# BaptisteHudyma/RGB-D-SLAM

Measured on AMD Instinct MI355X. Metric: depth frames/s primitive extraction (640x480), higher is better.
Workload: dtype f64; 1 GPU; 640x480 synthetic planar-room depth stream, plane extraction only (BASELINE.json configs[1]); stream_frames=4096, unique_frames_per_gpu=4096, scene=room, sub_batches=0, frames_rendered_on=device (torch)

## Files before the change

profiles/a1_inventory.py:

```python
#!/usr/bin/env python3
import argparse
import os
import re
import subprocess
import sys

sys.path.insert(0, os.path.dirname(os.path.abspath(__file__)))
from valu_issue import CSRC, RATE_NS, classify

SYMBOLS = (("f32", "_ZN4cape24cape_cell_moments_kernelILb0EEEvNS_12StageAParamsE"),
           ("u16", "_ZN4cape24cape_cell_moments_kernelILb1EEEvNS_12StageAParamsE"))
ORDER = ("prologue", "first trips", "loop trip", "last trips", "partial store", "reduce wave", "scan waves", "scan f64 redo", "aux store")
WEIGHT = {"prologue": 1, "first trips": 1, "loop trip": 3, "last trips": 1, "partial store": 1, "reduce wave": 0.2, "scan waves": 0.8,
          "scan f64 redo": 0.0, "aux store": 0.8}


def find(body, lo, pred):
    return next(i for i in range(lo, len(body)) if pred(body[i]))


def regions(asm, symbol):
    start = next(i for i, ln in enumerate(asm) if ln.startswith(symbol + ":"))
    end = find(asm, start, lambda ln: "s_endpgm" in ln)
    body = asm[start + 1:end + 1]
    is_depth_load = lambda ln: re.search(r"global_load_dwordx[24] .* nt$", ln.rstrip()) is not None
    first_load = find(body, 0, is_depth_load)
    head = find(body, 0, lambda ln: "Loop Header" in ln)
    label = body[head].split(":")[0]
    loop_end = find(body, head, lambda ln: re.search(r"s_c?branch\w*\s+" + re.escape(label) + r"\b", ln) is not None)
    skip = re.search(r"s_cbranch_execz\s+(\S+)", body[find(body, 0, lambda ln: "s_cbranch_execz" in ln)]).group(1)
    join = find(body, loop_end, lambda ln: ln.startswith(skip + ":"))
    barrier = find(body, join, lambda ln: "s_barrier" in ln)
    out = {"prologue": body[:first_load], "first trips": body[first_load:head], "loop trip": body[head:loop_end + 1],
           "last trips": body[loop_end + 1:join], "partial store": body[join:barrier + 1]}
    br = find(body, barrier, lambda ln: re.search(r"s_cbranch_\w+\s+\.LBB", ln) is not None)
    target = re.search(r"(\.LBB\w+)", body[br]).group(1)
    split = find(body, br, lambda ln: ln.startswith(target + ":"))
    arms = [body[barrier + 1:split], body[split:]]
    reduce_arm = next(a for a in arms if any("global_store_dwordx2" in ln for ln in a))
    scan_arm = next(a for a in arms if a is not reduce_arm)
    out["reduce wave"] = reduce_arm
    last_perm = max(i for i, ln in enumerate(scan_arm) if "ds_bpermute_b32" in ln)
    scan, redo = scan_arm[:last_perm + 1], []
    for i, ln in enumerate(scan):
        m = re.search(r"s_cbranch_vccz\s+(\.LBB\w+)", ln)
        if m:
            j = find(scan, i, lambda x: x.startswith(m.group(1) + ":"))
            if any(re.search(r"v_cmp_\w+_f64", x) for x in scan[i:j]):
                scan, redo = scan[:i + 1] + scan[j:], scan[i + 1:j]
                break
    out["scan waves"], out["scan f64 redo"], out["aux store"] = scan, redo, scan_arm[last_perm + 1:]
    return out


def count(lines):
    c = {"f64": 0, "double_rate": 0, "other": 0}
    for ln in lines:
        m = re.match(r"\s+(v_\w+)", ln)
        if m:
            c[classify(m.group(1))] += 1
    return c


def inventory(asm):
    res = {}
    for variant, symbol in SYMBOLS:
        res[variant] = {name: count(lines) for name, lines in regions(asm, symbol).items()}
    return res


def priced(c):
    return sum(c[k] * RATE_NS[k] for k in RATE_NS)


def main():
    ap = argparse.ArgumentParser()
    ap.add_argument("--asm", default="")
    args = ap.parse_args()
    path = args.asm
    if not path:
        path = "/tmp/cape_cell_moments.inventory.s"
        flags = "-O3 -std=c++17 -fPIC --offload-arch=gfx950 -ffp-contract=off -fno-fast-math -fno-slp-vectorize".split()
        subprocess.check_call(["/opt/rocm/bin/hipcc"] + flags + ["-S", "--cuda-device-only", "-o", path, os.path.join(CSRC, "cape_cell_moments.hip")],
                              stderr=subprocess.DEVNULL)
    inv = inventory(open(path).read().splitlines())
    for variant, regs in inv.items():
        print(f"{variant}   VALU instructions as listed                      f64-rate  double-rate  other   total   runs/wave   issue ns/wave")
        tot_n = tot_ns = 0.0
        for name in ORDER:
            c = regs[name]
            n = c["f64"] + c["double_rate"] + c["other"]
            ns = priced(c) * WEIGHT[name]
            tot_n += n * WEIGHT[name]
            tot_ns += ns
            print(f"  {name:<48} {c['f64']:8d} {c['double_rate']:12d} {c['other']:6d} {n:7d} {WEIGHT[name]:11.1f} {ns:15.1f}")
        print(f"  {'per wave, weighted':<48} {'':8} {'':12} {'':6} {tot_n:7.0f} {'':11} {tot_ns:15.1f}")


if __name__ == "__main__":
    main()
```

profiles/valu_issue.py:

```python
#!/usr/bin/env python3
import argparse
import csv
import json
import os
import re
import subprocess
import sys

ROOT = os.path.dirname(os.path.dirname(os.path.abspath(__file__)))
CSRC = os.path.join(ROOT, "rgb-d-slam_amd", "csrc")

RATE_NS = {"f64": 1.95, "other": 1.85, "double_rate": 0.95}
DOUBLE_RATE = {"v_mul_f32", "v_add_f32", "v_sub_f32", "v_subrev_f32", "v_add_u32", "v_sub_u32", "v_subrev_u32", "v_and_b32", "v_mov_b32"}


def classify(op):
    base = re.sub(r"_(e32|e64|dpp|sdwa)$", "", op)
    if "f64" in base or base.endswith("_b64") and base.startswith("v_mov"):
        return "f64"
    if base in DOUBLE_RATE:
        return "double_rate"
    return "other"


def kernel_regions(asm_lines, symbol):
    start = next(i for i, ln in enumerate(asm_lines) if ln.startswith(symbol + ":"))
    end = next(i for i in range(start, len(asm_lines)) if "s_endpgm" in asm_lines[i])
    body = asm_lines[start + 1:end + 1]
    loop_head = next(i for i, ln in enumerate(body) if "Loop Header" in ln)
    loop_label = body[loop_head].split(":")[0]
    loop_end = next(i for i in range(loop_head, len(body)) if re.search(r"s_c?branch\w*\s+" + re.escape(loop_label) + r"\b", body[i]))
    barrier = next(i for i in range(loop_end, len(body)) if "s_barrier" in body[i])

    def ops(lo, hi):
        out = []
        for ln in body[lo:hi]:
            m = re.match(r"\s+([vs]_\w+|ds_\w+|global_\w+|buffer_\w+|flat_\w+)", ln)
            if m:
                out.append(m.group(1))
        return out

    return [("first_trip", ops(0, loop_head)), ("rolled_trip", ops(loop_head, loop_end + 1)), ("last_trip", ops(loop_end + 1, barrier)),
            ("tail", ops(barrier, len(body)))]


def count(ops):
    c = {"f64": 0, "double_rate": 0, "other": 0, "salu": 0, "lds": 0, "vmem": 0}
    for op in ops:
        if op.startswith("v_"):
            c[classify(op)] += 1
        elif op.startswith("s_"):
            c["salu"] += 1
        elif op.startswith("ds_"):
            c["lds"] += 1
        else:
            c["vmem"] += 1
    return c


def main():
    ap = argparse.ArgumentParser()
    ap.add_argument("--pmc", default="")
    ap.add_argument("--frames", type=int, default=4096)
    ap.add_argument("--width", type=int, default=640)
    ap.add_argument("--height", type=int, default=480)
    ap.add_argument("--simds", type=int, default=1024)
    ap.add_argument("--out", default=os.path.join(ROOT, "profiles", "valu_issue.json"))
    args = ap.parse_args()

    asm_path = "/tmp/cape_cell_moments.gfx950.s"
    flags = "-O3 -std=c++17 -fPIC --offload-arch=gfx950 -ffp-contract=off -fno-fast-math -fno-slp-vectorize".split()
    subprocess.check_call(["/opt/rocm/bin/hipcc"] + flags + ["-S", "--cuda-device-only", "-o", asm_path, os.path.join(CSRC, "cape_cell_moments.hip")],
                          stderr=subprocess.DEVNULL)
    asm = open(asm_path).read().splitlines()
    rows_per_trip, cell = 4, 20
    trips = cell // rows_per_trip
    bands = (args.height // cell) * ((args.width + 639) // 640)
    waves_per_launch = args.frames * ((bands + 1) // 2) * 5
    out = {"kernel": "cape_cell_moments_kernel", "frames_per_launch": args.frames, "width": args.width, "height": args.height,
           "waves_per_launch": waves_per_launch, "simds": args.simds, "rate_ns_per_wave_instruction": RATE_NS,
           "rates_from": "profiles/r02_valu_rates.txt (csrc/microbench/valu_rates.hip on MI355X)", "variants": {}}
    for variant, symbol in (("f32", "_ZN4cape24cape_cell_moments_kernelILb0EEEvNS_12StageAParamsE"),
                            ("u16", "_ZN4cape24cape_cell_moments_kernelILb1EEEvNS_12StageAParamsE")):
        regs = dict(kernel_regions(asm, symbol))
        c = {k: count(v) for k, v in regs.items()}
        weights = {"first_trip": 1, "rolled_trip": trips - 2, "last_trip": 1}
        per_wave = {k: sum(c[r][k] * w for r, w in weights.items()) for k in ("f64", "double_rate", "other", "salu", "lds", "vmem")}
        tail_static = sum(c["tail"][k] for k in ("f64", "double_rate", "other"))
        v = {"static_per_wave": {"row_loop": per_wave, "tail_listed": c["tail"], "per_16_pixels_rolled_trip": c["rolled_trip"]}}
        loop_valu = per_wave["f64"] + per_wave["double_rate"] + per_wave["other"]
        tail_dyn = None
        if args.pmc:
            for row in csv.DictReader(open(args.pmc)):
                if ("cell_moments_kernel<false>" if variant == "f32" else "cell_moments_kernel<true>") in row["kernel"] and row["counter"] == "SQ_INSTS_VALU":
                    dyn = float(row["avg_value"])
                    v["pmc"] = {"SQ_INSTS_VALU_per_launch": dyn, "per_wave": dyn / waves_per_launch, "source": os.path.relpath(args.pmc, ROOT)}
                    tail_dyn = dyn / waves_per_launch - loop_valu
        if tail_dyn is None:
            tail_dyn = 0.5 * tail_static
            v["tail_note"] = "no PMC pass given: the tail is priced at half its listed instructions"
        else:
            v["tail_note"] = ("tail = SQ_INSTS_VALU per wave minus the row loop's static count: its blocks (partial-sum reduce on wave 4, "
                              "continuity scans on waves 0-3) run on subsets of the workgroup's waves")
        mix = {k: c["tail"][k] / max(1, tail_static) for k in ("f64", "double_rate", "other")}
        per_wave_ns = sum(per_wave[k] * RATE_NS[k] for k in RATE_NS) + tail_dyn * sum(mix[k] * RATE_NS[k] for k in RATE_NS)
        floor_ms = per_wave_ns * waves_per_launch / args.simds * 1e-6
        f64_ns = per_wave["f64"] * RATE_NS["f64"]
        v.update({"valu_per_wave": loop_valu + tail_dyn, "tail_valu_per_wave": tail_dyn, "issue_ns_per_wave": per_wave_ns, "floor_ms": floor_ms,
                  "f64_rate_share_of_floor": f64_ns / per_wave_ns,
                  "f64_rate_insts_per_launch": per_wave["f64"] * waves_per_launch,
                  "other_insts_per_launch": (per_wave["double_rate"] + per_wave["other"] + tail_dyn) * waves_per_launch})
        out["variants"][variant] = v
        print(f"{variant}: row loop per wave f64-rate {per_wave['f64']}, double-rate {per_wave['double_rate']}, other {per_wave['other']}; "
              f"tail {tail_dyn:.0f} (listed {tail_static}); issue floor {floor_ms:.3f} ms per {args.frames} frames "
              f"({100 * f64_ns / per_wave_ns:.0f} % of it the f64-rate instructions the reference's operand types dictate)", file=sys.stderr)
    json.dump(out, open(args.out, "w"), indent=1)
    print(args.out)


if __name__ == "__main__":
    main()
```

rgb-d-slam_amd/csrc/cape_api.hip:

```cpp
#include <algorithm>
#include <cmath>
#include <cstdlib>
#include <cstring>
#include <initializer_list>
#include <memory>
#include <new>
#include <random>
#include <string>
#include <vector>

#include "cape_handle.h"

using namespace cape::abi;

namespace {

thread_local std::string g_lastError;

constexpr int kRngTableMin = 40000;
int rng_table_size(int cells) { const int need = 43 * cells + 129; return need > kRngTableMin ? need : kRngTableMin; }

std::vector<double> rng_table(uint32_t seed, int count)
{
    std::vector<double> rng((size_t)count);
    std::mt19937 engine(seed);
    std::uniform_real_distribution<double> dist(0.0, 1.0);
    for (auto& v : rng)
        v = dist(engine);
    return rng;
}

void inverse_intrinsics(double fx, double fy, double cx, double cy, double& k00, double& k02, double& k11, double& k12)
{
    const double m[3][3] = {{fx, 0.0, cx}, {0.0, fy, cy}, {0.0, 0.0, 1.0}};
    auto cof = [&](int i, int j) {
        const int i1 = (i + 1) % 3, i2 = (i + 2) % 3, j1 = (j + 1) % 3, j2 = (j + 2) % 3;
        return m[i1][j1] * m[i2][j2] - m[i1][j2] * m[i2][j1];
    };
    const double c00 = cof(0, 0), c10 = cof(1, 0), c20 = cof(2, 0);
    const double det = (c00 * m[0][0] + c10 * m[1][0]) + c20 * m[2][0];
    const double invdet = 1.0 / det;
    k00 = c00 * invdet;
    k02 = c20 * invdet;
    k11 = cof(1, 1) * invdet;
    k12 = cof(2, 1) * invdet;
}

struct Knobs
{
    std::string resume;
    bool noResume = false;
    int schedule = 0;
    std::string stageA;
    bool growGeneral = false;
    bool pinnedByDma = false;
    int a2WideBatch = 0;
    int generalSlots = 0;
};

int read_knobs(Knobs& k)
{
    auto one_of = [](const char* name, std::initializer_list<const char*> values, std::string& out) {
        const char* e = std::getenv(name);
        if (!e)
            return true;
        out = e;
        return std::any_of(values.begin(), values.end(), [&](const char* v) { return out == v; });
    };
    std::string schedule, grow;
    if (!one_of("CAPE_RESUME", {"off", "wave", "group"}, k.resume))
        return fail(CAPE_ERR_INVALID_ARGUMENT, "CAPE_RESUME must be off, wave or group");
    if (!one_of("CAPE_SCHEDULE", {"two", "single"}, schedule))
        return fail(CAPE_ERR_INVALID_ARGUMENT, "CAPE_SCHEDULE must be two or single");
    if (!one_of("CAPE_STAGE_A", {"strips", "bands"}, k.stageA))
        return fail(CAPE_ERR_INVALID_ARGUMENT, "CAPE_STAGE_A must be strips or bands");
    if (!one_of("CAPE_GROW", {"general", "fast"}, grow))
        return fail(CAPE_ERR_INVALID_ARGUMENT, "CAPE_GROW must be general or fast");
    k.noResume = k.resume == "off" || std::getenv("CAPE_NO_RESUME");
    k.schedule = schedule == "two" ? 1 : (schedule == "single" ? 2 : 0);
    k.growGeneral = grow == "general";
    const char* e = std::getenv("CAPE_PINNED_INPUT");
    k.pinnedByDma = e && std::string(e) == "dma";
    if ((e = std::getenv("CAPE_A2_WIDE_BATCH")))
        k.a2WideBatch = std::atoi(e);
    if ((e = std::getenv("CAPE_GENERAL_SLOTS")))
        k.generalSlots = std::max(1, std::atoi(e));
    return CAPE_OK;
}

template <typename NextFn> int log_frame(cape_log_fn fn, void* user, const cape_frame_record& r, int frame, NextFn next)
{
    int lines = 0;
    const uint32_t st = r.header.status;
    for (uint32_t k = 0; k < CAPE_FRAME_NOT_PLANAR_COUNT(st); ++k, ++lines)
        fn(0, "Plane segment is not planar after merge", frame, user);
    if (st & CAPE_FRAME_INVALID_SEED)
        fn(1, "Could not find a single plane segment: invalid seed", frame, user), ++lines;
    int at = frame;
    for (const cape_frame_record* q = &r; q;)
    {
        const int n = q->header.n_plane_segments < CAPE_MAX_PLANES ? q->header.n_plane_segments : CAPE_MAX_PLANES;
        for (int i = 0; i < n; ++i)
        {
            const cape_plane_segment& s = q->segments[i];
            if (s.merge_label == (uint32_t)(i + q->header.segment_base) && s.planar && s.boundary_count < 3)
                fn(1, "Could not find a correct boundary polygon, rejecting plane segment", frame, user), ++lines;
        }
        const int nxt = q->header.next_record;
// ... 257 lines not shown
    CAPE_HIP_TRY(hipMemcpy(h->brow, brow.data(), brow.size() * sizeof(double), hipMemcpyHostToDevice));
    CAPE_HIP_TRY(hipMemcpy(h->ratioCol, rc.data(), rc.size() * sizeof(float), hipMemcpyHostToDevice));
    CAPE_HIP_TRY(hipMemcpy(h->ratioRow, rr.data(), rr.size() * sizeof(float), hipMemcpyHostToDevice));
    CAPE_HIP_TRY(hipMemcpy(h->rng, rng.data(), rng.size() * sizeof(double), hipMemcpyHostToDevice));
    if (h->resultsOnHost)
        std::memset(r.records, 0, R * sizeof(cape_frame_record));
    else
        CAPE_HIP_TRY(hipMemset(r.records, 0, R * sizeof(cape_frame_record)));

    cape::StageAParams& a = h->pa;
    a.W = cfg->width;
    a.H = cfg->height;
    a.hCells = h->hCells;
    a.vCells = h->vCells;
    a.cells = h->cells;
    a.segsPerRow = (h->hCells + 31) / 32;
    a.bandsPerFrame = h->vCells * a.segsPerRow;
    a.pairsPerFrame = (a.bandsPerFrame + 1) / 2;
    a.acol = h->acol;
    a.brow = h->brow;
    a.ratio_col = h->ratioCol;
    a.ratio_row = h->ratioRow;
    a.cell_sums = h->cellSums;
    a.cell_plane = h->cellPlane;
    a.cell_score = h->cellScore;
    a.cell_tol = h->cellTol;
    a.cell_flags = h->cellFlags;
    a.cell_bins = h->cellBins;
    a.cell_aux = h->cellAux;
    a.cell_mse = h->cellMse;
    a.sinMerge = sinf(static_cast<float>(18.0f * M_PI / 180.0));
    a.cosMergeA = std::cos(static_cast<double>(18.0f) * M_PI / 180.0);
    a.smallBatchFrames = knobs.a2WideBatch;
    a.minZeroPointCount = static_cast<int>(std::floor(static_cast<float>(400) * 0.7f));

    cape::StageBParams& b = h->pb;
    b.W = cfg->width;
    b.H = cfg->height;
    b.hCells = h->hCells;
    b.vCells = h->vCells;
    b.cells = h->cells;
    b.acol = h->acol;
    b.brow = h->brow;
    b.cell_sums = h->cellSums;
    b.cell_plane = h->cellPlane;
    b.cell_score = h->cellScore;
    b.cell_tol = h->cellTol;
    b.cell_flags = h->cellFlags;
    b.cell_bins = h->cellBins;
    b.cell_aux = h->cellAux;
    b.cell_mse = h->cellMse;
    b.records = r.records;
    b.plane_labels = r.planeLabels;
    b.cyl_labels = r.cylLabels;
    b.boundary = r.boundary;
    b.boundaryCapacity = h->boundaryCap;
    b.flags = cfg->flags;
    b.cosMerge = std::cos(static_cast<double>(18.0f) * M_PI / 180.0);
    b.planeSeedCount = static_cast<int>(static_cast<unsigned>((0.8 / 100.0) * h->cells));
    b.minCellActivated = static_cast<int>(static_cast<unsigned>((0.65 / 100.0) * h->cells));
    b.cylScratch = c.cylScratch;
    b.needCylinder = c.needCylinder;
    b.redoList = c.redoList;
    b.spillList = c.spillList;
    b.resumeList = c.resumeList;
    b.resumeBucketStride = c.resumeList ? (uint32_t)(2 * B + 2) : 0u;
// ... 222 lines not shown
```

rgb-d-slam_amd/csrc/cape_cell_acc.h:

```cpp
#pragma once
#include <hip/hip_runtime.h>

#include "cape_device.h"
#include "cape_internal.h"

namespace cape {


#ifndef CAPE_A_GROUP
#define CAPE_A_GROUP 2
#endif
#ifndef CAPE_A_WAVES
#define CAPE_A_WAVES 4
#endif

constexpr int kThreadsA = 320;
constexpr int kBandThreads = 160;
[[maybe_unused]] constexpr int kPartStride = 11;

struct PxAcc
{
    double S[9];
    uint32_t n;
    uint32_t zminBits1, zmaxBits;
};

__device__ __forceinline__ float acc_px(float zr, double a, double b, PxAcc& A)
{
    const bool valid = zr > 0.0f;
    const float z = valid ? zr : 0.0f;
    A.n += valid ? 1u : 0u;
    const double zd = (double)z;
    const float x = (float)(zd * a);
    const float y = (float)(zd * b);
    A.S[0] += (double)x;
    A.S[1] += (double)y;
    A.S[2] += zd;
    A.S[3] += (double)(x * x);
    A.S[4] += (double)(y * y);
    A.S[5] += (double)(z * z);
    A.S[6] += (double)(x * y);
    A.S[7] += (double)(y * z);
    A.S[8] += (double)(x * z);
    return z;
}

__device__ __forceinline__ uint32_t acc_px_fast(float z, double a, double b, PxAcc& A)
// ... 67 lines not shown
```

rgb-d-slam_amd/csrc/cape_cell_moments.hip:

```cpp
#include <hip/hip_runtime.h>

#include <type_traits>

#include "cape_cell_acc.h"

namespace cape {

template <bool U16> __global__ __launch_bounds__(kThreadsA, CAPE_A_WAVES) void cape_cell_moments_kernel(StageAParams p)
{
    __shared__ double s_part[kThreadsA * kPartStride];
    __shared__ float s_row[64 * kCell];
    __shared__ float s_col[64 * kCell];
    __shared__ float s_corner[64 * 2];
    __shared__ float s_trash[kThreadsA + kCell];

    const int t = threadIdx.x;
    const int frame = blockIdx.x / p.pairsPerFrame;
    const int pair = blockIdx.x - frame * p.pairsPerFrame;
    const size_t frameOff = (size_t)frame * p.W * p.H;

    const int band0 = pair * 2;
    const int cellRow0 = band0 / p.segsPerRow;
    const int seg0 = band0 - cellRow0 * p.segsPerRow;
    const bool wrap = seg0 + 1 == p.segsPerRow;
    const int cellRowOf[2] = {cellRow0, cellRow0 + (wrap ? 1 : 0)};
    const int segOf[2] = {seg0, wrap ? 0 : seg0 + 1};
    const bool bandExists[2] = {band0 < p.bandsPerFrame, band0 + 1 < p.bandsPerFrame};
    const int firstRowOf[2] = {__builtin_amdgcn_readfirstlane(cellRowOf[0] * kCell), __builtin_amdgcn_readfirstlane(cellRowOf[1] * kCell)};
    const int firstColOf[2] = {__builtin_amdgcn_readfirstlane(segOf[0] * 640), __builtin_amdgcn_readfirstlane(segOf[1] * 640)};
    const uint32_t firstPixOf[2] = {(uint32_t)__builtin_amdgcn_readfirstlane(firstRowOf[0] * p.W), (uint32_t)__builtin_amdgcn_readfirstlane(firstRowOf[1] * p.W)};
    const int colLimitOf[2] = {bandExists[0] ? p.W : 0, bandExists[1] ? p.W : 0};

    const int bsel = t / kBandThreads;
    const int q = t - bsel * kBandThreads;
    const int row0 = bsel ? firstRowOf[1] : firstRowOf[0];
    const int col0 = (bsel ? firstColOf[1] : firstColOf[0]) + q * 4;
    const bool active = col0 < (bsel ? colLimitOf[1] : colLimitOf[0]);
    const int cseg = q / 5;
    const int j = q - cseg * 5;
    const int lcell = bsel * 32 + cseg;

// ... 186 lines not shown
    const int fb = w >> 1, fs = (w & 1) * 16 + (l & 15);
    if ((l >> 4) != 0 || !(fb ? bandExists[1] : bandExists[0]))
        return;
    const int fRow = fb ? cellRowOf[1] : cellRowOf[0];
    const int fCol = (fb ? segOf[1] : segOf[0]) * 32 + fs;
    if (fCol >= p.hCells)
        return;
    uint32_t zminBits1 = 0xFFFFFFFFu, zmaxBits = 0u;
    uint32_t n = 0;
    {
        const int pbase = fb * kBandThreads + fs * 5;
#pragma unroll
        for (int k = 0; k < 5; ++k)
        {
            const uint2 zr = reinterpret_cast<const uint2*>(s_part + (pbase + k) * kPartStride + 10)[0];
            zminBits1 = min(zminBits1, zr.x);
            zmaxBits = max(zmaxBits, zr.y);
            n += (uint32_t)s_part[(pbase + k) * kPartStride + 9];
        }
    }
    const float zmin = __uint_as_float(zminBits1 + 1u), zmax = __uint_as_float(zmaxBits);
    const float rab = fmaxf(p.ratio_col[fCol], p.ratio_row[fRow]);
    const bool exact_ok = zmaxBits <= 0x7F7FFFFFu && ((n == 0) || (zmax * rab <= 512.0f * zmin));

    const size_t gcell = (size_t)frame * p.cells + fRow * p.hCells + fCol;
    CellAux aux;
    aux.z0 = s_corner[c64 * 2];
    aux.z399 = s_corner[c64 * 2 + 1];
    aux.flags = (n & kCountMask) | (continuous ? kAuxContinuous : 0u) | (exact_ok ? kAuxExact : 0u);
    aux.zc = s_row[c64 * kCell + kCell / 2];
    p.cell_aux[gcell] = aux;
}

hipError_t launch_cell_moments(const StageAParams& p, int nFrames, hipStream_t stream)
{
    const int grid = nFrames * p.pairsPerFrame;
    if (p.depth)
        hipLaunchKernelGGL(cape_cell_moments_kernel<false>, dim3(grid), dim3(kThreadsA), 0, stream, p);
    else
        hipLaunchKernelGGL(cape_cell_moments_kernel<true>, dim3(grid), dim3(kThreadsA), 0, stream, p);
    return hipGetLastError();
}

}
```

rgb-d-slam_amd/csrc/cape_grow.hip:

```cpp
#include <hip/hip_runtime.h>

#include "cape_grow_common.h"

namespace cape {

struct GrowLds
{
    size_t seg, chunk, adj, hist, bins, list, lab, mlab, cyl, ids, idmask, best, cur, dist, pendCyl, zc, prof, bytes;
};
__host__ __device__ inline GrowLds grow_lds(int cells, bool cylinders, int maxPlanes, bool resume)
{
    CAPE_LAYOUT_CHECK(cylinders || !resume);
    const size_t C = (size_t)cells;
    Layout l;
    GrowLds o{};
    o.seg = l.take<double>((size_t)(maxPlanes + 1) * kSegDoubles);
    o.chunk = l.take<double>(resume ? 0 : kChunkDoubles(cells));
    o.adj = l.take<unsigned long long>((size_t)maxPlanes + 1);
    o.hist = l.take<int>(resume ? 0 : kHistBins);
    o.bins = l.take<short>(resume ? 0 : C);
    o.list = l.take<unsigned short>(C + 4);
    o.lab = l.take<unsigned char>(C);
    o.mlab = l.take<unsigned char>((size_t)maxPlanes);
    if (cylinders)
// ... 391 lines not shown
            s_pendCyl[i] = g.seg[(hd.pendBaseSlot + hd.pendFrom) * kSegDoubles + i];
        if (lane < nRec)
            s_adj[lane] = g.adj[hd.pendFrom + lane];
        for (int i = lane; i < C + 4; i += 64)
            s_list[i] = g.list[i];
        for (int i = lane; i < C; i += 64)
        {
            s_lab[i] = g.lab[i];
            s_cyl[i] = 0;
        }
        pendCount = nRec;
        CAPE_WAVE_SYNC();
    }

    for (;;)
    {
        if (moreSeeds && !(untried > 0 && nSeeds < maxSeedIters))
            moreSeeds = false;
        if constexpr (!RESUME)
        if (moreSeeds)
            do
            {
                unsigned key = 0;
                for (int b = lane; b < kHistBins; b += 64)
                {
                    const int h = s_hist[b];
                    const unsigned k = ((unsigned)h << 16) | (unsigned)(0xFFFF - b);
                    key = (h > 0 && k > key) ? k : key;
                }
                key = wave_max_u32(key);
                if (key == 0)
                {
                    moreSeeds = false;
                    break;
                }
                const int bin = 0xFFFF - (int)(key & 0xFFFFu);
                CAPE_TICK(1);

                int candLocal = 0;
                unsigned long long bestLocal = ~0ull;
                int bestIdxLocal = 0x7FFFFFFF;
                if (mseInRegs)
                {
#pragma unroll
                    for (int k = 0; k < kMseRegs; ++k)
                    {
                        const int i = lane + 64 * k;
                        if (i < C && s_bins[i] == (short)bin)
                        {
                            ++candLocal;
                            const unsigned long long mb = (unsigned long long)__double_as_longlong(mreg[k]);
                            if (mb < bestLocal)
                            {
                                bestLocal = mb;
                                bestIdxLocal = i;
                            }
                        }
                    }
                }
                else
                {
                    constexpr int kBatch = 12;
                    for (int i0 = lane; i0 < C; i0 += 64 * kBatch)
                    {
                        double mv[kBatch];
#pragma unroll
                        for (int k = 0; k < kBatch; ++k)
                        {
                            const int i = i0 + 64 * k;
                            mv[k] = mseBase[i < C ? i : 0];
                        }
#pragma unroll
                        for (int k = 0; k < kBatch; ++k)
                        {
                            const int i = i0 + 64 * k;
                            if (i < C && s_bins[i] == (short)bin)
                            {
                                ++candLocal;
                                const unsigned long long mb = (unsigned long long)__double_as_longlong(mv[k]);
                                if (mb < bestLocal)
                                {
                                    bestLocal = mb;
                                    bestIdxLocal = i;
                                }
                            }
                        }
                    }
                }
                CAPE_TICK(2);
                const int cand = wave_sum_i32(candLocal);
                if (cand < p.planeSeedCount || cand == 0)
                {
                    moreSeeds = false;
                    break;
                }
                const unsigned long long bestAll = wave_min_u64(bestLocal);
                const unsigned idxKey = (bestLocal == bestAll) ? (unsigned)(0x7FFFFFFF - bestIdxLocal) : 0u;
                const int seed = 0x7FFFFFFF - (int)wave_max_u32(idxKey);
                if (__longlong_as_double((long long)bestAll) >= kDblMax)
                {
                    moreSeeds = false;
                    status |= CAPE_FRAME_INVALID_SEED;
                    break;
                }
                if (lane == 0 && p.seed_sequence && nSeeds < C)
                    p.seed_sequence[cellBase + nSeeds] = (uint16_t)seed;
                ++nSeeds;

                const int sy = seed / HC, sx = seed - sy * HC;
                const double2* spl = reinterpret_cast<const double2*>(p.cell_plane + (cellBase + seed) * kPlaneStride);
                const double2 sp0 = spl[0], sp1 = spl[1], sp2 = spl[2], sp3 = spl[3];
                const float stolf = p.cell_tol[cellBase + seed];
                const MaskT seedRowU = shfl_mask<MaskT>(U, sy);
                const bool seedUnassigned = test_bit<MaskT>(seedRowU, sx);

                CAPE_TICK(3);
                MaskT act = 0;
                if (seedUnassigned)
                {
                    if (lane == sy)
                        act = (MaskT)1 << sx;
                    for (;;)
                    {
                        MaskT a = act;
                        for (;;)
                        {
// ... 459 lines not shown
```

rgb-d-slam_amd/csrc/cape_grow_general.hip:

```cpp
#include <cstdlib>

#include <hip/hip_runtime.h>

#include "cape_grow_common.h"

namespace cape {

namespace {

using Lab = unsigned short;
using u64 = unsigned long long;
constexpr int kGenPend = 64;

struct GenDims
{
    int C, HC, VC, Wd, items, capSeg, capCyl, chainMax;
    bool cyl;
};

struct GenPtrs
{
    u64 *U, *L2M, *M2L, *U2M, *M2U;
    u64 *act;
    u64 *T0, *T1;
// ... 221 lines not shown
                }
            }
        }
    }
    const int nPlanar = wave_sum_i32(nPlanarLocal);
    CAPE_WAVE_SYNC();

    int untried = nPlanar;
    int nSeg = 0, nCylLabels = 0, nCylFits = 0, rngPos = 0, nSeeds = 0;
    const double* sumsBase = p.cell_sums + cellBase * kSumStride;
    const double* mseBase = p.cell_mse + cellBase;
    const int maxSeedIters = 4 * C + 1024;
    int pendCount = 0, listTop = 0;
    bool moreSeeds = true, stopAll = false;

    for (;;)
    {
        if (moreSeeds && !(untried > 0 && nSeeds < maxSeedIters))
            moreSeeds = false;
        if (moreSeeds)
            do
            {
                unsigned key = 0;
                for (int b = lane; b < kHistBins; b += 64)
                {
                    const int h = s_hist[b];
                    const unsigned k = ((unsigned)h << 16) | (unsigned)(0xFFFF - b);
                    key = (h > 0 && k > key) ? k : key;
                }
                key = wave_max_u32(key);
                if (key == 0)
                {
                    moreSeeds = false;
                    break;
                }
                const int bin = 0xFFFF - (int)(key & 0xFFFFu);

                int candLocal = 0;
                u64 bestLocal = ~0ull;
                int bestIdxLocal = 0x7FFFFFFF;
                {
                    constexpr int kBatch = 8;
                    for (int i0 = lane; i0 < C; i0 += 64 * kBatch)
                    {
                        double mv[kBatch];
#pragma unroll
                        for (int k = 0; k < kBatch; ++k)
                        {
                            const int i = i0 + 64 * k;
                            mv[k] = mseBase[i < C ? i : 0];
                        }
#pragma unroll
                        for (int k = 0; k < kBatch; ++k)
                        {
                            const int i = i0 + 64 * k;
                            if (i < C && P.bins[i] == (short)bin)
                            {
                                ++candLocal;
                                const u64 mb = (u64)__double_as_longlong(mv[k]);
                                if (mb < bestLocal)
                                {
                                    bestLocal = mb;
                                    bestIdxLocal = i;
                                }
                            }
                        }
                    }
                }
                const int cand = wave_sum_i32(candLocal);
                if (cand < p.planeSeedCount || cand == 0)
                {
                    moreSeeds = false;
                    break;
                }
                const u64 bestAll = wave_min_u64(bestLocal);
                const unsigned idxKey = (bestLocal == bestAll) ? (unsigned)(0x7FFFFFFF - bestIdxLocal) : 0u;
                const int seed = 0x7FFFFFFF - (int)wave_max_u32(idxKey);
                if (__longlong_as_double((long long)bestAll) >= kDblMax)
                {
                    moreSeeds = false;
                    status |= CAPE_FRAME_INVALID_SEED;
                    break;
                }
                if (lane == 0 && p.seed_sequence && nSeeds < C)
                    p.seed_sequence[cellBase + nSeeds] = (uint16_t)seed;
                ++nSeeds;

                const int sy = seed / HC, sx = seed - sy * HC;
                const double2* spl = reinterpret_cast<const double2*>(p.cell_plane + (cellBase + seed) * kPlaneStride);
                const double2 sp0 = spl[0], sp1 = spl[1], sp2 = spl[2], sp3 = spl[3];
                const float stolf = p.cell_tol[cellBase + seed];
                const int seedItem = sy * Wd + (sx >> 6);
                const bool seedUnassigned = (P.U[seedItem] >> (sx & 63)) & 1ull;

                for (int it = lane; it < items; it += 64)
                    P.act[it] = 0ull;
                CAPE_WAVE_SYNC();
                bool seedOK;
                {
                    const double snx = sp0.x, sny = sp0.y, snz = sp1.x, sd = sp1.y, scx = sp2.x, scy = sp2.y, scz = sp3.x;
                    double pnx = snx, pny = sny, pnz = snz;
                    normalize3(pnx, pny, pnz);
                    seedOK = can_be_merged(pnx, pny, pnz, sd, snx, sny, snz, scx, scy, scz, (double)stolf, p.cosMerge);
                }
                if (seedUnassigned && seedOK)
// ... 729 lines not shown
```

rgb-d-slam_amd/csrc/cape_internal.h:

```cpp
#pragma once
#include <stdint.h>

#include "../../include/cape_hip.h"

namespace cape {

constexpr int kSumStride = 10;
constexpr int kFastPlanes = 32;
constexpr int kProfileSlots = 32;
constexpr int kResumeClasses = 8;
constexpr int kCylStride = 8;
constexpr int kPlaneStride = 8;
constexpr uint32_t kFlagPlanar = 1u << 31;
constexpr uint32_t kFlagInorder = 1u << 30;
constexpr uint32_t kFlagNearEdge = 1u << 29;
constexpr uint32_t kCountMask = (1u << 24) - 1;
constexpr uint32_t kFlagLeftToMe = 1u << 24;
constexpr uint32_t kFlagMeToLeft = 1u << 25;
constexpr uint32_t kFlagUpToMe = 1u << 26;
constexpr uint32_t kFlagMeToUp = 1u << 27;
constexpr uint32_t kAuxContinuous = 1u << 31;
constexpr uint32_t kAuxExact = 1u << 30;

struct CellAux
// ... 3 lines not shown
    float zc;
};

struct StageAParams
{
    const float* depth;
    const uint16_t* depth_u16;
    float u16_scale;
    int W, H, hCells, vCells, cells;
    int segsPerRow;
    int bandsPerFrame;
    int pairsPerFrame;
    const double* acol;
    const double* brow;
    const float* ratio_col;
    const float* ratio_row;
    double* cell_sums;
    double* cell_plane;
    double* cell_score;
    float* cell_tol;
    uint32_t* cell_flags;
    int32_t* cell_bins;
    CellAux* cell_aux;
    double* cell_mse;
    float sinMerge;
    uint32_t* clear0;
    uint32_t* clear1;
    uint32_t* clear2;
    uint32_t clear2Buckets;
    uint32_t* clear3;
    uint32_t* clear4;
    double cosMergeA;
    int smallBatchFrames;
    int minZeroPointCount;
};

struct StageBParams
{
    int W, H, hCells, vCells, cells;
    const double* acol;
    const double* brow;
    const double* cell_sums;
    const double* cell_plane;
    const double* cell_score;
    const float* cell_tol;
    const uint32_t* cell_flags;
    const int32_t* cell_bins;
    const CellAux* cell_aux;
    const double* cell_mse;
    cape_frame_record* records;
    int32_t* plane_labels;
    int32_t* cyl_labels;
    double* boundary;
    int boundaryCapacity;
    uint32_t flags;
    double cosMerge;
    int planeSeedCount;
    int minCellActivated;
    const double* rngTable;
    int rngCount;
    int ransacMaxIterations;
    double* cylScratch;
    uint32_t* needCylinder;
    uint32_t* redoList;
    uint32_t* spillList;
    uint32_t* resumeList;
// ... 323 lines not shown
```

Before: 2.343 million frames/s.

## Add one-cell-per-lane moments kernel as default stage A1 path

Adds a new cell-moments kernel in which each lane accumulates one whole 20x20 cell, streaming its rows through buffer loads with register prefetch. It replaces the band kernel, which used shared-memory partial sums, a barrier and a reduce/scan tail across waves; that kernel stays reachable through CAPE_A1=bands. Continuity scans for the centre row and column run inline per lane. The trade is more registers per lane and strided per-lane memory access in exchange for no LDS reduction. Seed-status flag handling in the grow kernels and the profiling scripts are updated alongside.

```diff
diff --git a/profiles/a1_inventory.py b/profiles/a1_inventory.py
--- a/profiles/a1_inventory.py
+++ b/profiles/a1_inventory.py
@@ -1,72 +1,30 @@
 #!/usr/bin/env python3
 import argparse
 import os
-import re
 import subprocess
 import sys
 
 sys.path.insert(0, os.path.dirname(os.path.abspath(__file__)))
-from valu_issue import CSRC, RATE_NS, classify
+from valu_issue import CSRC, RATE_NS, classify, kernel_regions
 
-SYMBOLS = (("f32", "_ZN4cape24cape_cell_moments_kernelILb0EEEvNS_12StageAParamsE"),
-           ("u16", "_ZN4cape24cape_cell_moments_kernelILb1EEEvNS_12StageAParamsE"))
-ORDER = ("prologue", "first trips", "loop trip", "last trips", "partial store", "reduce wave", "scan waves", "scan f64 redo", "aux store")
-WEIGHT = {"prologue": 1, "first trips": 1, "loop trip": 3, "last trips": 1, "partial store": 1, "reduce wave": 0.2, "scan waves": 0.8,
-          "scan f64 redo": 0.0, "aux store": 0.8}
+SYMBOLS = (("f32", "_ZN4cape24cape_cell_moments_kernelILb0EEEvNS_12StageAParamsEi"),
+           ("u16", "_ZN4cape24cape_cell_moments_kernelILb1EEEvNS_12StageAParamsEi"))
+NAMES = {"prologue": "prologue", "loop_rows_0_9": "rows 0..9, one trip", "row_10": "row 10", "loop_rows_11_18": "rows 11..18, one trip",
+         "tail": "tail", "redo_listed": "scan f64 redo"}
+ORDER = tuple(NAMES)
+WEIGHT = {"prologue": 1, "loop_rows_0_9": 10, "row_10": 1, "loop_rows_11_18": 8, "tail": 1, "redo_listed": 0}
 
 
-def find(body, lo, pred):
-    return next(i for i in range(lo, len(body)) if pred(body[i]))
-
-
-def regions(asm, symbol):
-    start = next(i for i, ln in enumerate(asm) if ln.startswith(symbol + ":"))
-    end = find(asm, start, lambda ln: "s_endpgm" in ln)
-    body = asm[start + 1:end + 1]
-    is_depth_load = lambda ln: re.search(r"global_load_dwordx[24] .* nt$", ln.rstrip()) is not None
-    first_load = find(body, 0, is_depth_load)
-    head = find(body, 0, lambda ln: "Loop Header" in ln)
-    label = body[head].split(":")[0]
-    loop_end = find(body, head, lambda ln: re.search(r"s_c?branch\w*\s+" + re.escape(label) + r"\b", ln) is not None)
-    skip = re.search(r"s_cbranch_execz\s+(\S+)", body[find(body, 0, lambda ln: "s_cbranch_execz" in ln)]).group(1)
-    join = find(body, loop_end, lambda ln: ln.startswith(skip + ":"))
-    barrier = find(body, join, lambda ln: "s_barrier" in ln)
-    out = {"prologue": body[:first_load], "first trips": body[first_load:head], "loop trip": body[head:loop_end + 1],
-           "last trips": body[loop_end + 1:join], "partial store": body[join:barrier + 1]}
-    br = find(body, barrier, lambda ln: re.search(r"s_cbranch_\w+\s+\.LBB", ln) is not None)
-    target = re.search(r"(\.LBB\w+)", body[br]).group(1)
-    split = find(body, br, lambda ln: ln.startswith(target + ":"))
-    arms = [body[barrier + 1:split], body[split:]]
-    reduce_arm = next(a for a in arms if any("global_store_dwordx2" in ln for ln in a))
-    scan_arm = next(a for a in arms if a is not reduce_arm)
-    out["reduce wave"] = reduce_arm
-    last_perm = max(i for i, ln in enumerate(scan_arm) if "ds_bpermute_b32" in ln)
-    scan, redo = scan_arm[:last_perm + 1], []
-    for i, ln in enumerate(scan):
-        m = re.search(r"s_cbranch_vccz\s+(\.LBB\w+)", ln)
-        if m:
-            j = find(scan, i, lambda x: x.startswith(m.group(1) + ":"))
-            if any(re.search(r"v_cmp_\w+_f64", x) for x in scan[i:j]):
-                scan, redo = scan[:i + 1] + scan[j:], scan[i + 1:j]
-                break
-    out["scan waves"], out["scan f64 redo"], out["aux store"] = scan, redo, scan_arm[last_perm + 1:]
-    return out
-
-
-def count(lines):
+def count(ops):
     c = {"f64": 0, "double_rate": 0, "other": 0}
-    for ln in lines:
-        m = re.match(r"\s+(v_\w+)", ln)
-        if m:
-            c[classify(m.group(1))] += 1
+    for op in ops:
+        if op.startswith("v_"):
+            c[classify(op)] += 1
     return c
 
 
 def inventory(asm):
-    res = {}
-    for variant, symbol in SYMBOLS:
-        res[variant] = {name: count(lines) for name, lines in regions(asm, symbol).items()}
-    return res
+    return {variant: {name: count(ops) for name, ops in kernel_regions(asm, symbol)} for variant, symbol in SYMBOLS}
 
 
 def priced(c):
@@ -93,8 +51,9 @@
             ns = priced(c) * WEIGHT[name]
             tot_n += n * WEIGHT[name]
             tot_ns += ns
-            print(f"  {name:<48} {c['f64']:8d} {c['double_rate']:12d} {c['other']:6d} {n:7d} {WEIGHT[name]:11.1f} {ns:15.1f}")
-        print(f"  {'per wave, weighted':<48} {'':8} {'':12} {'':6} {tot_n:7.0f} {'':11} {tot_ns:15.1f}")
+            print(f"  {NAMES[name]:<48} {c['f64']:8d} {c['double_rate']:12d} {c['other']:6d} {n:7d} {WEIGHT[name]:11.1f} {ns:15.1f}")
+        print(f"  {'per wave (64 cells), weighted':<48} {'':8} {'':12} {'':6} {tot_n:7.0f} {'':11} {tot_ns:15.1f}")
+        print(f"  {'per 80 pixels per lane (the band instance: 2 790)':<48} {'':8} {'':12} {'':6} {tot_n / 5:7.0f} {'':11} {tot_ns / 5:15.1f}")
 
 
 if __name__ == "__main__":
diff --git a/profiles/valu_issue.py b/profiles/valu_issue.py
--- a/profiles/valu_issue.py
+++ b/profiles/valu_issue.py
@@ -27,21 +27,38 @@
     start = next(i for i, ln in enumerate(asm_lines) if ln.startswith(symbol + ":"))
     end = next(i for i in range(start, len(asm_lines)) if "s_endpgm" in asm_lines[i])
     body = asm_lines[start + 1:end + 1]
-    loop_head = next(i for i, ln in enumerate(body) if "Loop Header" in ln)
-    loop_label = body[loop_head].split(":")[0]
-    loop_end = next(i for i in range(loop_head, len(body)) if re.search(r"s_c?branch\w*\s+" + re.escape(loop_label) + r"\b", body[i]))
-    barrier = next(i for i in range(loop_end, len(body)) if "s_barrier" in body[i])
+    label_at = {m.group(1): i for i, ln in enumerate(body) for m in [re.match(r"^(\.LBB\d+_\d+):", ln)] if m}
+    loops = []
+    for i, ln in enumerate(body):
+        m = re.match(r"\s+s_c?branch\w*\s+(\.LBB\d+_\d+)", ln)
+        if m and label_at.get(m.group(1), len(body)) < i:
+            loops.append((label_at[m.group(1)], i))
+    assert len(loops) == 2, "two row loops"
+    redo = []
 
     def ops(lo, hi):
-        out = []
+        out, skip_to = [], None
         for ln in body[lo:hi]:
-            m = re.match(r"\s+([vs]_\w+|ds_\w+|global_\w+|buffer_\w+|flat_\w+)", ln)
+            if skip_to is not None:
+                if ln.startswith(skip_to + ":"):
+                    skip_to = None
+                else:
+                    m = re.match(r"\s+([vs]_\w+)", ln)
+                    if m:
+                        redo.append(m.group(1))
+                    continue
+            m = re.match(r"\s+([vs]_\w+|ds_\w+|global_\w+|buffer_\w+|flat_\w+|scratch_\w+)", ln)
             if m:
                 out.append(m.group(1))
+                v = re.match(r"\s+s_cbranch_vccz\s+(\.LBB\d+_\d+)", ln)
+                if v:
+                    skip_to = v.group(1)
         return out
 
-    return [("first_trip", ops(0, loop_head)), ("rolled_trip", ops(loop_head, loop_end + 1)), ("last_trip", ops(loop_end + 1, barrier)),
-            ("tail", ops(barrier, len(body)))]
+    (h1, e1), (h2, e2) = loops
+    regions = [("prologue", ops(0, h1)), ("loop_rows_0_9", ops(h1, e1 + 1)), ("row_10", ops(e1 + 1, h2)), ("loop_rows_11_18", ops(h2, e2 + 1)),
+               ("tail", ops(e2 + 1, len(body)))]
+    return regions + [("redo_listed", redo)]
 
 
 def count(ops):
@@ -73,46 +90,40 @@
     subprocess.check_call(["/opt/rocm/bin/hipcc"] + flags + ["-S", "--cuda-device-only", "-o", asm_path, os.path.join(CSRC, "cape_cell_moments.hip")],
                           stderr=subprocess.DEVNULL)
     asm = open(asm_path).read().splitlines()
-    rows_per_trip, cell = 4, 20
-    trips = cell // rows_per_trip
-    bands = (args.height // cell) * ((args.width + 639) // 640)
-    waves_per_launch = args.frames * ((bands + 1) // 2) * 5
+    cell = 20
+    cells = (args.height // cell) * (args.width // cell)
+    waves_per_launch = args.frames * ((cells + 63) // 64)
     out = {"kernel": "cape_cell_moments_kernel", "frames_per_launch": args.frames, "width": args.width, "height": args.height,
            "waves_per_launch": waves_per_launch, "simds": args.simds, "rate_ns_per_wave_instruction": RATE_NS,
            "rates_from": "profiles/r02_valu_rates.txt (csrc/microbench/valu_rates.hip on MI355X)", "variants": {}}
-    for variant, symbol in (("f32", "_ZN4cape24cape_cell_moments_kernelILb0EEEvNS_12StageAParamsE"),
-                            ("u16", "_ZN4cape24cape_cell_moments_kernelILb1EEEvNS_12StageAParamsE")):
+    for variant, symbol in (("f32", "_ZN4cape24cape_cell_moments_kernelILb0EEEvNS_12StageAParamsEi"),
+                            ("u16", "_ZN4cape24cape_cell_moments_kernelILb1EEEvNS_12StageAParamsEi")):
         regs = dict(kernel_regions(asm, symbol))
         c = {k: count(v) for k, v in regs.items()}
-        weights = {"first_trip": 1, "rolled_trip": trips - 2, "last_trip": 1}
+        weights = {"prologue": 1, "loop_rows_0_9": cell // 2, "row_10": 1, "loop_rows_11_18": cell // 2 - 2, "tail": 1}
         per_wave = {k: sum(c[r][k] * w for r, w in weights.items()) for k in ("f64", "double_rate", "other", "salu", "lds", "vmem")}
-        tail_static = sum(c["tail"][k] for k in ("f64", "double_rate", "other"))
-        v = {"static_per_wave": {"row_loop": per_wave, "tail_listed": c["tail"], "per_16_pixels_rolled_trip": c["rolled_trip"]}}
-        loop_valu = per_wave["f64"] + per_wave["double_rate"] + per_wave["other"]
-        tail_dyn = None
+        static_valu = per_wave["f64"] + per_wave["double_rate"] + per_wave["other"]
+        v = {"static_per_wave": {"all_rows": per_wave, "per_region": {r: c[r] for r in weights}, "redo_listed_not_run": c["redo_listed"],
+                                 "per_20_pixels_row_trip": c["loop_rows_0_9"]}}
+        valu = static_valu
         if args.pmc:
             for row in csv.DictReader(open(args.pmc)):
                 if ("cell_moments_kernel<false>" if variant == "f32" else "cell_moments_kernel<true>") in row["kernel"] and row["counter"] == "SQ_INSTS_VALU":
                     dyn = float(row["avg_value"])
-                    v["pmc"] = {"SQ_INSTS_VALU_per_launch": dyn, "per_wave": dyn / waves_per_launch, "source": os.path.relpath(args.pmc, ROOT)}
-                    tail_dyn = dyn / waves_per_launch - loop_valu
-        if tail_dyn is None:
-            tail_dyn = 0.5 * tail_static
-            v["tail_note"] = "no PMC pass given: the tail is priced at half its listed instructions"
-        else:
-            v["tail_note"] = ("tail = SQ_INSTS_VALU per wave minus the row loop's static count: its blocks (partial-sum reduce on wave 4, "
-                              "continuity scans on waves 0-3) run on subsets of the workgroup's waves")
-        mix = {k: c["tail"][k] / max(1, tail_static) for k in ("f64", "double_rate", "other")}
-        per_wave_ns = sum(per_wave[k] * RATE_NS[k] for k in RATE_NS) + tail_dyn * sum(mix[k] * RATE_NS[k] for k in RATE_NS)
+                    v["pmc"] = {"SQ_INSTS_VALU_per_launch": dyn, "per_wave": dyn / waves_per_launch, "static_per_wave": static_valu,
+                                "source": os.path.relpath(args.pmc, ROOT)}
+                    valu = dyn / waves_per_launch
+        mix = {k: per_wave[k] / max(1, static_valu) for k in RATE_NS}
+        per_wave_ns = valu * sum(mix[k] * RATE_NS[k] for k in RATE_NS)
         floor_ms = per_wave_ns * waves_per_launch / args.simds * 1e-6
-        f64_ns = per_wave["f64"] * RATE_NS["f64"]
-        v.update({"valu_per_wave": loop_valu + tail_dyn, "tail_valu_per_wave": tail_dyn, "issue_ns_per_wave": per_wave_ns, "floor_ms": floor_ms,
+        f64_ns = valu * mix["f64"] * RATE_NS["f64"]
+        v.update({"valu_per_wave": valu, "issue_ns_per_wave": per_wave_ns, "floor_ms": floor_ms,
                   "f64_rate_share_of_floor": f64_ns / per_wave_ns,
-                  "f64_rate_insts_per_launch": per_wave["f64"] * waves_per_launch,
-                  "other_insts_per_launch": (per_wave["double_rate"] + per_wave["other"] + tail_dyn) * waves_per_launch})
+                  "f64_rate_insts_per_launch": valu * mix["f64"] * waves_per_launch,
+                  "other_insts_per_launch": valu * (1.0 - mix["f64"]) * waves_per_launch})
         out["variants"][variant] = v
-        print(f"{variant}: row loop per wave f64-rate {per_wave['f64']}, double-rate {per_wave['double_rate']}, other {per_wave['other']}; "
-              f"tail {tail_dyn:.0f} (listed {tail_static}); issue floor {floor_ms:.3f} ms per {args.frames} frames "
+        print(f"{variant}: per wave (64 cells) f64-rate {per_wave['f64']}, double-rate {per_wave['double_rate']}, other {per_wave['other']} "
+              f"= {static_valu} listed, {valu:.0f} priced ({valu / 5:.0f} per 80 pixels per lane); issue floor {floor_ms:.3f} ms per {args.frames} frames "
               f"({100 * f64_ns / per_wave_ns:.0f} % of it the f64-rate instructions the reference's operand types dictate)", file=sys.stderr)
     json.dump(out, open(args.out, "w"), indent=1)
     print(args.out)
diff --git a/rgb-d-slam_amd/csrc/cape_api.hip b/rgb-d-slam_amd/csrc/cape_api.hip
--- a/rgb-d-slam_amd/csrc/cape_api.hip
+++ b/rgb-d-slam_amd/csrc/cape_api.hip
@@ -52,6 +52,7 @@
     bool noResume = false;
     int schedule = 0;
     std::string stageA;
+    std::string a1;
     bool growGeneral = false;
     bool pinnedByDma = false;
     int a2WideBatch = 0;
@@ -74,6 +75,8 @@
         return fail(CAPE_ERR_INVALID_ARGUMENT, "CAPE_SCHEDULE must be two or single");
     if (!one_of("CAPE_STAGE_A", {"strips", "bands"}, k.stageA))
         return fail(CAPE_ERR_INVALID_ARGUMENT, "CAPE_STAGE_A must be strips or bands");
+    if (!one_of("CAPE_A1", {"cells", "bands"}, k.a1))
+        return fail(CAPE_ERR_INVALID_ARGUMENT, "CAPE_A1 must be cells or bands");
     if (!one_of("CAPE_GROW", {"general", "fast"}, grow))
         return fail(CAPE_ERR_INVALID_ARGUMENT, "CAPE_GROW must be general or fast");
     k.noResume = k.resume == "off" || std::getenv("CAPE_NO_RESUME");
@@ -397,6 +400,7 @@
     a.sinMerge = sinf(static_cast<float>(18.0f * M_PI / 180.0));
     a.cosMergeA = std::cos(static_cast<double>(18.0f) * M_PI / 180.0);
     a.smallBatchFrames = knobs.a2WideBatch;
+    a.a1Bands = knobs.a1 == "bands" ? 1 : 0;
     a.minZeroPointCount = static_cast<int>(std::floor(static_cast<float>(400) * 0.7f));
 
     cape::StageBParams& b = h->pb;
diff --git a/rgb-d-slam_amd/csrc/cape_cell_acc.h b/rgb-d-slam_amd/csrc/cape_cell_acc.h
--- a/rgb-d-slam_amd/csrc/cape_cell_acc.h
+++ b/rgb-d-slam_amd/csrc/cape_cell_acc.h
@@ -13,6 +13,18 @@
 #ifndef CAPE_A_WAVES
 #define CAPE_A_WAVES 4
 #endif
+
+#ifndef CAPE_A1_CELL_WAVES
+#define CAPE_A1_CELL_WAVES 4
+#endif
+#ifndef CAPE_A1_CELL_THREADS
+#define CAPE_A1_CELL_THREADS 256
+#endif
+#ifndef CAPE_A1_CELL_LOAD_POLICY
+#define CAPE_A1_CELL_LOAD_POLICY 0
+#endif
+constexpr int kThreadsCells = CAPE_A1_CELL_THREADS;
+static_assert(kThreadsCells % 64 == 0 && kThreadsCells >= 64 && kThreadsCells <= 1024, "whole waves");
 
 constexpr int kThreadsA = 320;
 constexpr int kBandThreads = 160;
diff --git a/rgb-d-slam_amd/csrc/cape_cell_moments.hip b/rgb-d-slam_amd/csrc/cape_cell_moments.hip
--- a/rgb-d-slam_amd/csrc/cape_cell_moments.hip
+++ b/rgb-d-slam_amd/csrc/cape_cell_moments.hip
@@ -6,7 +6,7 @@
 
 namespace cape {
 
-template <bool U16> __global__ __launch_bounds__(kThreadsA, CAPE_A_WAVES) void cape_cell_moments_kernel(StageAParams p)
+template <bool U16> __global__ __launch_bounds__(kThreadsA, CAPE_A_WAVES) void cape_cell_moments_bands_kernel(StageAParams p)
 {
     __shared__ double s_part[kThreadsA * kPartStride];
     __shared__ float s_row[64 * kCell];
@@ -259,13 +259,218 @@
     p.cell_aux[gcell] = aux;
 }
 
+template <bool U16> __global__ __launch_bounds__(kThreadsCells, CAPE_A1_CELL_WAVES) void cape_cell_moments_kernel(StageAParams p, int nWaves)
+{
+    const int gw = __builtin_amdgcn_readfirstlane((int)(blockIdx.x * (kThreadsCells / 64) + (threadIdx.x >> 6)));
+    if (gw >= nWaves)
+        return;
+    const int wavesPerFrame = (p.cells + 63) >> 6;
+    const int frame = gw / wavesPerFrame;
+    const int w = gw - frame * wavesPerFrame;
+    const int cell = w * 64 + (int)(threadIdx.x & 63);
+    if (cell >= p.cells)
+        return;
+    const int cellRow = cell / p.hCells;
+    const int cellCol = cell - cellRow * p.hCells;
+    const size_t frameOff = (size_t)frame * p.W * p.H;
+
+    PxAcc A;
+#pragma unroll
+    for (int k = 0; k < 9; ++k)
+        A.S[k] = 0.0;
+    A.n = 0;
+    A.zminBits1 = 0xFFFFFFFFu;
+    A.zmaxBits = 0u;
+
+    double a[kCell];
+    {
+        const double2* ap = reinterpret_cast<const double2*>(p.acol + cellCol * kCell);
+#pragma unroll
+        for (int k = 0; k < kCell / 2; ++k)
+        {
+            const double2 v = ap[k];
+            a[2 * k] = v.x;
+            a[2 * k + 1] = v.y;
+        }
+    }
+    auto acc_piece = [&](const float4& v, int j, double b) { acc_f4(v, a[4 * j], a[4 * j + 1], a[4 * j + 2], a[4 * j + 3], b, A); };
+
+    constexpr uint32_t kPixBytes = U16 ? 2 : 4;
+    const uint32_t pixByteOff = ((uint32_t)(cellRow * kCell) * (uint32_t)p.W + (uint32_t)(cellCol * kCell)) * kPixBytes;
+    const uint32_t browByteOff = (uint32_t)(cellRow * kCell) * 8u;
+    const uint32_t rowBytes = (uint32_t)p.W * kPixBytes;
+    const float scale16 = p.u16_scale;
+    auto uniform_ptr = [](const void* q) {
+        const uint64_t u = reinterpret_cast<uint64_t>(q);
+        const uint32_t lo = __builtin_amdgcn_readfirstlane((uint32_t)u), hi = __builtin_amdgcn_readfirstlane((uint32_t)(u >> 32));
+        return reinterpret_cast<void*>(((uint64_t)hi << 32) | lo);
+    };
+    const void* frameBase = U16 ? (const void*)(p.depth_u16 + frameOff) : (const void*)(p.depth + frameOff);
+    const __amdgpu_buffer_rsrc_t frameRsrc =
+        __builtin_amdgcn_make_buffer_rsrc(uniform_ptr(frameBase), 0, (int)((uint32_t)p.H * rowBytes), 0x00020000);
+    const __amdgpu_buffer_rsrc_t browRsrc = __builtin_amdgcn_make_buffer_rsrc(uniform_ptr(p.brow), 0, p.H * 8, 0x00020000);
+    auto brow_at = [&](int r) {
+        typedef uint32_t u32x2 __attribute__((ext_vector_type(2)));
+        const u32x2 v = __builtin_amdgcn_raw_buffer_load_b64(browRsrc, browByteOff, r * 8, 0);
+        return __hiloint2double((int)v.y, (int)v.x);
+    };
+
+    using Raw = typename std::conditional<U16, ushort4, float4>::type;
+    constexpr int kQuads = kCell / 4;
+    static_assert(kCell == 20, "five float4 per row, pixel column 10 = .z of piece 2");
+    auto load_piece = [&](int r, int j) -> Raw {
+        const int rowOff = r * (int)rowBytes;
+        if constexpr (U16)
+        {
+            typedef uint32_t u32x2 __attribute__((ext_vector_type(2)));
+            const u32x2 v = __builtin_amdgcn_raw_buffer_load_b64(frameRsrc, pixByteOff, rowOff + 8 * j, CAPE_A1_CELL_LOAD_POLICY);
+            return make_ushort4((unsigned short)(v.x & 0xFFFFu), (unsigned short)(v.x >> 16), (unsigned short)(v.y & 0xFFFFu), (unsigned short)(v.y >> 16));
+        }
+        else
+        {
+            typedef uint32_t u32x4 __attribute__((ext_vector_type(4)));
+            const u32x4 v = __builtin_amdgcn_raw_buffer_load_b128(frameRsrc, pixByteOff, rowOff + 16 * j, CAPE_A1_CELL_LOAD_POLICY);
+            return make_float4(__uint_as_float(v.x), __uint_as_float(v.y), __uint_as_float(v.z), __uint_as_float(v.w));
+        }
+    };
+    auto to_f4 = [&](const Raw& rw) {
+        if constexpr (U16)
+            return make_float4((float)rw.x * scale16, (float)rw.y * scale16, (float)rw.z * scale16, (float)rw.w * scale16);
+        else
+            return rw;
+    };
+
+    auto scan_step = [](float z, float& last, bool& continuous, bool counts) {
+        const float before = last;
+        bool unsure = false;
+        bool pass = is_continuous_flat_f32(z, last, unsure);
+        if (__any(unsure & counts))
+        {
+            last = before;
+            pass = is_continuous_flat(z, last);
+        }
+        continuous &= pass | !counts;
+    };
+    bool continuous = true;
+    auto my_cell = [&]() {
+        uint32_t lane = __builtin_amdgcn_mbcnt_hi(~0u, __builtin_amdgcn_mbcnt_lo(~0u, 0u));
+        asm volatile("" : "+v"(lane));
+        return ((size_t)frame * p.cells + (size_t)(w * 64)) + lane;
+    };
+
+    Raw buf[kQuads];
+#pragma unroll
+    for (int j = 0; j < kQuads; ++j)
+        buf[j] = load_piece(0, j);
+    double b = brow_at(0);
+    const float z0 = to_f4(buf[0]).x;
+    float zc = 0.0f;
+    float vLast = 0.0f;
+    auto stream_row = [&](int r) {
+        const double bn = brow_at(r + 1);
+        float zv = 0.0f;
+#pragma unroll
+        for (int j = 0; j < kQuads; ++j)
+        {
+            const float4 v = to_f4(buf[j]);
+            buf[j] = load_piece(r + 1, j);
+            acc_piece(v, j, b);
+            if (j == 2)
+                zv = v.z;
+        }
+        b = bn;
+        const float seed = std_maxf(vLast, zv);
+        vLast = r == 0 ? zv : (r == 1 ? seed : vLast);
+        continuous &= (r != 1) | !(vLast <= 0);
+        scan_step(zv, vLast, continuous, r != 0);
+    };
+#pragma unroll 1
+    for (int r = 0; r < kCell / 2; ++r)
+        stream_row(r);
+    {
+        const int r = kCell / 2;
+        float hLast = 0.0f;
+#pragma unroll
+        for (int j = 0; j < kQuads; ++j)
+        {
+            const float4 v = to_f4(buf[j]);
+            buf[j] = load_piece(r + 1, j);
+            acc_piece(v, j, b);
+            if (j == 0)
+            {
+                hLast = std_maxf(v.x, v.y);
+                continuous &= !(hLast <= 0);
+            }
+            else
+            {
+                scan_step(v.x, hLast, continuous, true);
+            }
+            scan_step(v.y, hLast, continuous, true);
+            scan_step(v.z, hLast, continuous, true);
+            scan_step(v.w, hLast, continuous, true);
+            if (j == 2)
+            {
+                zc = v.z;
+                scan_step(v.z, vLast, continuous, true);
+            }
+        }
+        b = brow_at(r + 1);
+    }
+#pragma unroll 1
+    for (int r = kCell / 2 + 1; r < kCell - 1; ++r)
+        stream_row(r);
+    float z399;
+#pragma unroll
+    for (int j = 0; j < kQuads; ++j)
+    {
+        const float4 v = to_f4(buf[j]);
+        acc_piece(v, j, b);
+        z399 = v.w;
+    }
+
+    const uint32_t n = A.n;
+    const float zmin = __uint_as_float(A.zminBits1 + 1u), zmax = __uint_as_float(A.zmaxBits);
+    const size_t gcell = my_cell();
+    const int ecell = (int)(gcell - (size_t)frame * p.cells);
+    int hCells = p.hCells;
+    asm volatile("" : "+s"(hCells));
+    const int eRow = ecell / hCells;
+    const float rab = fmaxf(p.ratio_col[ecell - eRow * hCells], p.ratio_row[eRow]);
+    const bool exact_ok = A.zmaxBits <= 0x7F7FFFFFu && ((n == 0) || (zmax * rab <= 512.0f * zmin));
+
+    CellAux aux;
+    aux.z0 = z0;
+    aux.z399 = z399;
+    aux.flags = (n & kCountMask) | (continuous ? kAuxContinuous : 0u) | (exact_ok ? kAuxExact : 0u);
+    aux.zc = zc;
+    p.cell_aux[gcell] = aux;
+    double2* dst = reinterpret_cast<double2*>(p.cell_sums + gcell * kSumStride);
+    static_assert(kSumStride == 10, "nine sums and the count: five 16-B stores");
+    dst[0] = make_double2(A.S[0], A.S[1]);
+    dst[1] = make_double2(A.S[2], A.S[3]);
+    dst[2] = make_double2(A.S[4], A.S[5]);
+    dst[3] = make_double2(A.S[6], A.S[7]);
+    dst[4] = make_double2(A.S[8], (double)n);
+}
+
 hipError_t launch_cell_moments(const StageAParams& p, int nFrames, hipStream_t stream)
 {
-    const int grid = nFrames * p.pairsPerFrame;
+    if (p.a1Bands)
+    {
+        const int grid = nFrames * p.pairsPerFrame;
+        if (p.depth)
+            hipLaunchKernelGGL(cape_cell_moments_bands_kernel<false>, dim3(grid), dim3(kThreadsA), 0, stream, p);
+        else
+            hipLaunchKernelGGL(cape_cell_moments_bands_kernel<true>, dim3(grid), dim3(kThreadsA), 0, stream, p);
+        return hipGetLastError();
+    }
+    constexpr int kWaves = kThreadsCells / 64;
+    const int waves = nFrames * ((p.cells + 63) / 64);
+    const int grid = (waves + kWaves - 1) / kWaves;
     if (p.depth)
-        hipLaunchKernelGGL(cape_cell_moments_kernel<false>, dim3(grid), dim3(kThreadsA), 0, stream, p);
+        hipLaunchKernelGGL(cape_cell_moments_kernel<false>, dim3(grid), dim3(kThreadsCells), 0, stream, p, waves);
     else
-        hipLaunchKernelGGL(cape_cell_moments_kernel<true>, dim3(grid), dim3(kThreadsA), 0, stream, p);
+        hipLaunchKernelGGL(cape_cell_moments_kernel<true>, dim3(grid), dim3(kThreadsCells), 0, stream, p, waves);
     return hipGetLastError();
 }
 
diff --git a/rgb-d-slam_amd/csrc/cape_grow.hip b/rgb-d-slam_amd/csrc/cape_grow.hip
--- a/rgb-d-slam_amd/csrc/cape_grow.hip
+++ b/rgb-d-slam_amd/csrc/cape_grow.hip
@@ -447,6 +447,8 @@
                 if (key == 0)
                 {
                     moreSeeds = false;
+                    if (p.planeSeedCount == 0)
+                        status |= CAPE_FRAME_INVALID_SEED;
                     break;
                 }
                 const int bin = 0xFFFF - (int)(key & 0xFFFFu);
@@ -507,6 +509,8 @@
                 if (cand < p.planeSeedCount || cand == 0)
                 {
                     moreSeeds = false;
+                    if (cand >= p.planeSeedCount)
+                        status |= CAPE_FRAME_INVALID_SEED;
                     break;
                 }
                 const unsigned long long bestAll = wave_min_u64(bestLocal);
diff --git a/rgb-d-slam_amd/csrc/cape_grow_general.hip b/rgb-d-slam_amd/csrc/cape_grow_general.hip
--- a/rgb-d-slam_amd/csrc/cape_grow_general.hip
+++ b/rgb-d-slam_amd/csrc/cape_grow_general.hip
@@ -277,6 +277,8 @@
                 if (key == 0)
                 {
                     moreSeeds = false;
+                    if (p.planeSeedCount == 0)
+                        status |= CAPE_FRAME_INVALID_SEED;
                     break;
                 }
                 const int bin = 0xFFFF - (int)(key & 0xFFFFu);
@@ -316,6 +318,8 @@
                 if (cand < p.planeSeedCount || cand == 0)
                 {
                     moreSeeds = false;
+                    if (cand >= p.planeSeedCount)
+                        status |= CAPE_FRAME_INVALID_SEED;
                     break;
                 }
                 const u64 bestAll = wave_min_u64(bestLocal);
diff --git a/rgb-d-slam_amd/csrc/cape_internal.h b/rgb-d-slam_amd/csrc/cape_internal.h
--- a/rgb-d-slam_amd/csrc/cape_internal.h
+++ b/rgb-d-slam_amd/csrc/cape_internal.h
@@ -59,6 +59,7 @@
     uint32_t* clear4;
     double cosMergeA;
     int smallBatchFrames;
+    int a1Bands;
     int minZeroPointCount;
 };
 
```

Measured after the change: 2.553 million frames/s (median of 6 runs). 1.09x the previous value.
